# ami-iit/paper_gorbani_2025_humanoids_multi-rate-mpc-ironcub

Measured on AMD Instinct MI355X. Metric: MPC solves/sec (whole node) + p50 single-solve latency, iRonCub paper horizon, higher is better.
Workload: dtype f64

## Files before the change

paper_gorbani_2025_humanoids_multi-rate-mpc-ironcub_amd/csrc/vsmpc_p1_struct.hpp:

```cpp
#pragma once
#include "vsmpc_smem.hpp"

namespace vsmpc {

VS_DEV double uniform_f64(double x) {
    const int lo = __builtin_amdgcn_readfirstlane(__double2loint(x));
    const int hi = __builtin_amdgcn_readfirstlane(__double2hiint(x));
    return __hiloint2double(hi, lo);
}

template <class D, int KIND, bool SMALL = false>
VS_DEV void p1s_chain(const DevCfg& cfg, int half, int lane, double* __restrict__ sm) {
    using S = Smem<D, SMALL>;
    constexpr int N = D::N, HC = D::HC, NV = D::NV;
    const double* sA = sm + S::oA;
    const double* sCfg = sm + S::oCfg;
    double* sH = sm + S::oSH;
    double* sRb = sm + S::oSRb;
    double* sW3 = sm + S::oSW3;
    const int xr0 = half ? 6 : 0, hr0 = half ? 9 : 3, er0 = half ? 23 : 20;
    const int yx0 = half ? 6 : 0, yh0 = half ? 9 : 3, ye0 = half ? 15 : 12;
    double M1[9], qx[3], qh[3], qe[3];
#pragma unroll
    for (int r = 0; r < 3; ++r) {
// ... 120 lines not shown
                for (int r = 0; r < 3; ++r) {
                    rf_n[r] = refRow[rc * 12 + yx0 + r + zo];
                    rf_n[3 + r] = refRow[rc * 12 + yh0 + r + zo];
                }
            }
        }
        if (m < N) {
            const double dtm = cfg.dt[m];
            double t[3];
#pragma unroll
            for (int r = 0; r < 3; ++r) t[r] = fma(M1[6 + r], nx[2], fma(M1[3 + r], nx[1], M1[r] * nx[0]));
            t[0] = fma(-s02, nh[2], fma(-s01, nh[1], t[0]));
            t[1] = fma(-s12, nh[2], fma(s01, nh[0], t[1]));
            t[2] = fma(s12, nh[1], fma(s02, nh[0], t[2]));
#pragma unroll
            for (int r = 0; r < 3; ++r) {
                nx[r] = fma(dtm, ne[r], nx[r]);
                nh[r] = fma(dtm, t[r], nh[r]);
            }
        }
#pragma unroll
        for (int r = 0; r < 3; ++r) {
            nx[r] = fma(qx[r], KIND == 1 ? x[r] - rf[r] : x[r], nx[r]);
            nh[r] = fma(qh[r], KIND == 1 ? hk[i][r] - rf[3 + r] : hk[i][r], nh[r]);
            ne[r] = fma(qe[r], e[r], ne[r]);
        }
        const double dti = cfg.dt[i];
        if (m >= 2) {
            double hp[3] = {hk[i - 1][0], hk[i - 1][1], hk[i - 1][2]};
            asm volatile("" : "+v"(hp[0]), "+v"(hp[1]), "+v"(hp[2]));
#pragma unroll
            for (int r = 0; r < 3; ++r) {
                const double dxr = fma(M1[3 * r + 2], hp[2], fma(M1[3 * r + 1], hp[1], M1[3 * r] * hp[0]));
                x[r] = fma(-dti, dxr, x[r]);
                e[r] = fma(-dti, x[r], e[r]);
            }
        }
        double w[3];
#pragma unroll
        for (int a = 0; a < 3; ++a) { w[a] = dti * nh[a]; bs[a] += w[a]; }
        if constexpr (KIND == 1 && !LONG) {
            if (i >= 1 && live) {
                double* Wp = sW3 + ((half * (NV + 1) + col) * (N - 1) + (i - 1)) * 3;
#pragma unroll
                for (int a = 0; a < 3; ++a) Wp[a] = w[a];
            }
        }
        if constexpr (KIND == 1 && LONG) {
            if (i >= 1) {
                if (live && !isgen && i - 1 >= acFirst) {
                    typedef __attribute__((address_space(3))) double lds_double;
                    double* Ap = sm + S::oSAc + acOff + (i - 1) * 4;
#pragma unroll
                    for (int q = 0; q < NTH; ++q) {
                        const double v = fma(Am[2][q], w[2], fma(Am[1][q], w[1], Am[0][q] * w[0]));
                        __builtin_amdgcn_ds_atomic_fadd_f64((lds_double*)(Ap + q), v, 0, 0, false);
                    }
                }
            }
        }
        if (i < HC) {
            if (isgen) {
                if (live && i >= gb) {
                    double* Hp = sH + (half * D::NJPAIR + i * (i + 1) / 2 + gb) * 9 + gd;
#pragma unroll
                    for (int a = 0; a < 3; ++a) Hp[3 * a] = bs[a];
                }
            } else {
                if (live) {
                    double* Rp = sRb + ((half * (NV + 1) + col) * HC + i) * 3;
#pragma unroll
                    for (int a = 0; a < 3; ++a) Rp[a] = bs[a];
                }
            }
#pragma unroll
            for (int a = 0; a < 3; ++a) bs[a] = 0.0;
        }
        asm volatile("" : "+v"(nx[0]), "+v"(nx[1]), "+v"(nx[2]), "+v"(nh[0]), "+v"(nh[1]), "+v"(nh[2]), "+v"(ne[0]), "+v"(ne[1]), "+v"(ne[2]));
        asm volatile("" : "+v"(x[0]), "+v"(x[1]), "+v"(x[2]), "+v"(e[0]), "+v"(e[1]), "+v"(e[2]), "+v"(bs[0]), "+v"(bs[1]), "+v"(bs[2]));
        __builtin_amdgcn_sched_barrier(0);
    }
}

template <class D, bool SMALL = false>
VS_DEV void p1s_contract(double* __restrict__ sm, int tid) {
    using S = Smem<D, SMALL>;
    constexpr int NI = (D::NV + 1) * (D::N - 1);
    constexpr int ROUNDS = (NI + D::BLOCK - 1) / D::BLOCK;
    const double* sA = sm + S::oA;
    const double* sW3 = sm + S::oSW3;
    double* sAc = sm + S::oSAc;
    double w[ROUNDS][6];
#pragma unroll
    for (int rd = 0; rd < ROUNDS; ++rd) {
        const int ci = tid + rd * D::BLOCK, cic = ci < NI ? ci : NI - 1;
#pragma unroll
        for (int a = 0; a < 3; ++a) { w[rd][a] = sW3[cic * 3 + a]; w[rd][3 + a] = sW3[(NI + cic) * 3 + a]; }
    }
    double Am[6][NTH];
#pragma unroll
    for (int a = 0; a < 3; ++a)
#pragma unroll
        for (int q = 0; q < NTH; ++q) { Am[a][q] = sA[(3 + a) * NX + 12 + q]; Am[3 + a][q] = sA[(9 + a) * NX + 12 + q]; }
#pragma unroll
    for (int rd = 0; rd < ROUNDS; ++rd) {
        const int ci = tid + rd * D::BLOCK;
        double v[NTH];
#pragma unroll
        for (int q = 0; q < NTH; ++q) {
            v[q] = Am[0][q] * w[rd][0];
#pragma unroll
            for (int a = 1; a < 6; ++a) v[q] = fma(Am[a][q], w[rd][a], v[q]);
        }
        if (ci < NI) {
#pragma unroll
            for (int q = 0; q < NTH; ++q) sAc[ci * 4 + q] = v[q];
        }
    }
}

template <class D, int TPW, int W, bool PIPE>
struct AllSlots {
    static constexpr bool SMALL = false;
    static constexpr int count = TPW;
    static constexpr int slot(int a) { return a; }
    static constexpr bool forms(int q) { return TileTab<D, PIPE>{}.forms(q * D::NWAVES + W, W); }
};
template <class D, int TPW, int W, bool PIPE = false, class PLAN = AllSlots<D, TPW, W, PIPE>>
VS_DEV void p1s_entries(d4 (&acc)[TPW], const double* __restrict__ sm, int lane) {
    using S = Smem<D, PLAN::SMALL>;
    constexpr int PVT = D::PVT, N = D::N, HC = D::HC, NV = D::NV;
    static_assert(D::NU % 16 == 0, "joint rows are tile aligned");
    const double* sBj = sm + S::oBj;
    const double* sH = sm + S::oSH;
    const double* sRb = sm + S::oSRb;
    const double* sAc = sm + S::oSAc;
    const double* sJetT = sm + S::oJetT;
    lane = fresh_lane();
    const int j = lane & 15, g = lane >> 4;
    double Lq[3][NJC], LqM[3][NJC];
    int bin[3];
#pragma unroll
    for (int pat = 0; pat < 3; ++pat) {
        const int o = ((16 * pat) % NJC) + j;
        bin[pat] = o / NJC;
        const int un = o - NJC * bin[pat];
#pragma unroll
        for (int a6 = 0; a6 < NJC; ++a6) {
            Lq[pat][a6] = sBj[((a6 < 3 ? 3 : 6) + a6) * NJ + un];
            LqM[pat][a6] = bin[pat] == g ? Lq[pat][a6] : 0.0;
        }
    }
    constexpr int G = 3;
    constexpr int NSLOT = PLAN::count;
    constexpr int NGRP = (NSLOT + G - 1) / G;
    static_for<0, NGRP>([&](auto gcst) __attribute__((always_inline)) {
    constexpr int q0 = decltype(gcst)::value * G;
    constexpr int q1 = q0 + G < NSLOT ? q0 + G : NSLOT;
    double raw[G][NJC][3];
    static_for<q0, q1>([&](auto qcst) __attribute__((always_inline)) {
        constexpr TileTab<D, PIPE> tab{};
        constexpr int qi = decltype(qcst)::value;
        constexpr int q = PLAN::slot(qi);
        constexpr int t = q * D::NWAVES + W;
        if constexpr (PLAN::forms(q)) {
            constexpr int ti = tab.ti[t], tj = tab.tj[t];
            if constexpr (ti < PVT) {
                constexpr int b0r = (16 * ti) / NJC, b0c = (16 * tj) / NJC;
                const int brr = b0r + g, bcc = b0c + bin[tj % 3];
                const int br = brr < HC ? brr : HC - 1, bc = bcc < HC ? bcc : HC - 1;
                const bool sw = ti == tj && br < bc;
                const int hi = sw ? bc : br, lo = sw ? br : bc;
                const int st = sw ? 3 : 1, sa = sw ? 1 : 3;
                const double* Hp = sH + (hi * (hi + 1) / 2 + lo) * 9;
#pragma unroll
                for (int ks = 0; ks < NJC; ++ks) {
                    const double* Hk = Hp + (ks / 3) * D::NJPAIR * 9 + sa * (ks % 3);
#pragma unroll
                    for (int d = 0; d < 3; ++d) raw[qi - q0][ks][d] = Hk[d * st];
                }
            } else if constexpr (tj < PVT) {
                constexpr int b0c = (16 * tj) / NJC;
                const int cr = 16 * (ti - PVT) + j;
                const int crc = cr <= NV ? cr : NV;
                const int bcc = b0c + g, bc = bcc < HC ? bcc : HC - 1;
#pragma unroll
                for (int ks = 0; ks < NJC; ++ks)
                    raw[qi - q0][ks][0] = sRb[(((ks / 3) * (NV + 1) + crc) * HC + bc) * 3 + (ks % 3)];
            }
        }
    });
    __builtin_amdgcn_sched_barrier(0);
    double opa[G][NJC], opb[G][NJC];
    static_for<q0, q1>([&](auto qcst) __attribute__((always_inline)) {
        constexpr TileTab<D, PIPE> tab{};
        constexpr int qi = decltype(qcst)::value;
        constexpr int q = PLAN::slot(qi);
        constexpr int t = q * D::NWAVES + W;
#pragma unroll
        for (int ks = 0; ks < NJC; ++ks) { opa[qi - q0][ks] = 0.0; opb[qi - q0][ks] = 0.0; }
// ... 99 lines not shown
```

paper_gorbani_2025_humanoids_multi-rate-mpc-ironcub_amd/csrc/vsmpc_p3.hpp:

```cpp
#pragma once
#include "vsmpc_p1_struct.hpp"
#include "vsmpc_smem.hpp"

namespace vsmpc {

template <class D>
VS_DEV double input_cost_term(const double* __restrict__ sCfg, const double* __restrict__ sGy,
                              const double* __restrict__ sVprev, int gr, int gc) {
    if (gr < D::NU) return (gr == gc) ? 1.0 : 0.0;
    if (gr < D::NZ) {
        if (gc < D::NU) return 0.0;
        const int q1 = gr - D::NU, q2 = gc - D::NU;
        if ((q1 & 3) != (q2 & 3)) return 0.0;
        const int b1 = v_block_of_internal<D>(q1), b2 = v_block_of_internal<D>(q2);
        if (b1 == b2)
            return sCfg[CFG_WTHR] * double((b1 > 0) + (b1 < D::NVB - 1)) + (b1 == 0 ? sCfg[CFG_WINIT] : 0.0);
        const int db = b1 - b2;
        return (db == 1 || db == -1) ? -sCfg[CFG_WTHR] : 0.0;
    }
    if (gr == D::NZ && gc < D::NZ) {
        if (gc < D::NU) return gc < D::NUY ? sGy[gc % NJC] : 0.0;
        const int q = gc - D::NU;
        return v_block_of_internal<D>(q) == 0 ? -sCfg[CFG_WINIT] * sVprev[q & 3] : 0.0;
    }
// ... 264 lines not shown
                for (int ks = 0; ks < 4; ++ks)
                    acc[q0] = __builtin_amdgcn_mfma_f64_16x16x4f64(la[b][0][ks], lb[b][0][ks], acc[q0], 0, 0, 0);
            } else {
                d4 c2 = d4{0.0, 0.0, 0.0, 0.0};
                acc[q0] = __builtin_amdgcn_mfma_f64_16x16x4f64(la[b][0][0], lb[b][0][0], acc[q0], 0, 0, 0);
                c2 = __builtin_amdgcn_mfma_f64_16x16x4f64(la[b][0][1], lb[b][0][1], c2, 0, 0, 0);
                acc[q0] = __builtin_amdgcn_mfma_f64_16x16x4f64(la[b][0][2], lb[b][0][2], acc[q0], 0, 0, 0);
                c2 = __builtin_amdgcn_mfma_f64_16x16x4f64(la[b][0][3], lb[b][0][3], c2, 0, 0, 0);
#pragma unroll
                for (int r = 0; r < 4; ++r) acc[q0][r] += c2[r];
            }
            if constexpr (KIND != 2) {
                static_for<0, 2>([&](auto ucst) __attribute__((always_inline)) {
                    constexpr int u = decltype(ucst)::value;
                    if constexpr (a + u < n) {
                        constexpr int q = u ? q1 : q0;
                        double* T = sM + tile_off_c<D>(tab.ti[q * D::NWAVES + W], PP + 1) + crow;
#pragma unroll
                        for (int r = 0; r < 4; ++r) T[4 * r * 17] = acc[q][r];
                    }
                });
            }
        }
    });
}

VS_DEV void tile_inverse_dpp(const double* __restrict__ Lpp, const double* __restrict__ invd, double* __restrict__ X, int lane) {
    panel_inverse_dpp(lds_addr(Lpp + (lane & 15) * 17), lds_addr(invd), lds_addr(X + (lane & 15)), lane & 15);
}

template <class D, int TPW>
constexpr int pipe_inverse_wave(int p) {
    constexpr WaveLists<D, TPW, 1, true> w1{};
    constexpr WaveLists<D, TPW, 2, true> w2{};
    constexpr WaveLists<D, TPW, 3, true> w3{};
    const int n1 = w1.nrest[p - 1], n2 = w2.nrest[p - 1], n3 = w3.nrest[p - 1];
    return (n3 <= n1 && n3 <= n2) ? 3 : (n2 <= n1 ? 2 : 1);
}

template <class D, int TPW, int W, bool PIPE, class PLAN>
VS_DEV void p2_terms(const double* __restrict__ sCfg, d4 (&acc)[TPW], const double* __restrict__ sGy,
                     const double* __restrict__ sVprev, int lane) {
    constexpr TileTab<D, PIPE> tab{};
    constexpr int PVT = D::PVT;
    static_for<0, PLAN::count>([&](auto qcst) __attribute__((always_inline)) {
        constexpr int q = PLAN::slot(decltype(qcst)::value);
        constexpr int t = q * D::NWAVES + W;
        if constexpr (PLAN::forms(q)) {
            constexpr int ti = tab.ti[t], tj = tab.tj[t];
            if constexpr (ti == tj && 16 * ti + 16 <= D::NU) {
#pragma unroll
                for (int r = 0; r < 4; ++r) acc[q][r] += ((lane >> 4) + 4 * r == (lane & 15)) ? 1.0 : 0.0;
            } else if constexpr (ti >= PVT && 16 * tj + 16 <= D::NU) {
                if constexpr (ti == D::NT - 1) {
                    const int gc = 16 * tj + (lane & 15);
                    const double gv = sGy[gc % NJC];
                    const double gq = gc < D::NUY ? gv : 0.0;
#pragma unroll
                    for (int r = 0; r < 4; ++r) acc[q][r] += (16 * ti + (lane >> 4) + 4 * r == D::NZ) ? gq : 0.0;
                }
            } else if constexpr (ti == tj || ti >= PVT) {
#pragma unroll
                for (int r = 0; r < 4; ++r)
                    acc[q][r] += input_cost_term<D>(sCfg, sGy, sVprev, 16 * ti + (lane >> 4) + 4 * r, 16 * tj + (lane & 15));
            }
        }
    });
}

constexpr int SMALL_BESIDE0 = 4;
template <class D>
constexpr bool small_wave0_forms(int ti) {
    return ti % (D::NWAVES - 1) == 0 && ti / (D::NWAVES - 1) < (D::NT + 1) / 4;
}
template <class D, int TPW, int W>
constexpr int small_instalment(int q) {
    constexpr TileTab<D, true> tab{};
    const int t = q * D::NWAVES + W;
    if (!tab.ok(t)) return -1;
    if (W == 0) return small_wave0_forms<D>(tab.ti[t]) ? 0 : -1;
    if (tab.tj[t] == 0) return (W == 1 && small_wave0_forms<D>(tab.ti[t])) ? -1 : 0;
    int n = 0;
    for (int b = 0; b < q; ++b) n += (tab.ok(b * D::NWAVES + W) && tab.tj[b * D::NWAVES + W] > 0) ? 1 : 0;
    return (tab.tj[t] == 1 || n < SMALL_BESIDE0) ? 1 : 2;
}
template <class D, int TPW, int W, int INST>
struct SmallPlan {
    static constexpr bool SMALL = true;
    static constexpr int count_() {
        int n = 0;
        for (int q = 0; q < TPW; ++q) n += small_instalment<D, TPW, W>(q) == INST ? 1 : 0;
        return n;
    }
    static constexpr int count = count_();
    static constexpr int slot(int a) {
        for (int q = 0; q < TPW; ++q)
            if (small_instalment<D, TPW, W>(q) == INST && a-- == 0) return q;
        return 0;
    }
    static constexpr bool forms(int) { return true; }
};
template <class D, int TPW>
constexpr bool small_plan_complete() {
    constexpr TileTab<D, true> tab{};
    int col0[D::NT] = {};
    for (int q = 0; q < TPW; ++q) {
        const int i0 = small_instalment<D, TPW, 0>(q);
        if (i0 >= 0) col0[tab.ti[q * D::NWAVES]] += 1;
        const int inst[3] = {small_instalment<D, TPW, 1>(q), small_instalment<D, TPW, 2>(q), small_instalment<D, TPW, 3>(q)};
        for (int w = 1; w < D::NWAVES; ++w) {
            const int t = q * D::NWAVES + w;
            if (!tab.ok(t)) continue;
            if (tab.tj[t] == 0) col0[tab.ti[t]] += inst[w - 1] == 0 ? 1 : 0;
            else if (inst[w - 1] < 1) return false;
        }
    }
    for (int i = 0; i < D::NT; ++i)
        if (col0[i] != 1) return false;
    return true;
}
template <class D, int TPW, int W, int INST>
VS_DEV void small_form(const double* __restrict__ sCfg, d4 (&acc)[TPW], double* __restrict__ sM, const double* __restrict__ sGy,
                       const double* __restrict__ sVprev, int lane, int crow) {
    using PLAN = SmallPlan<D, TPW, W, INST>;
    static_assert(small_plan_complete<D, TPW>(), "every tile is formed exactly once");
    if constexpr (PLAN::count > 0) {
        p1s_entries<D, TPW, W, true, PLAN>(acc, sM - Smem<D>::oM, lane);
        p2_terms<D, TPW, W, true, PLAN>(sCfg, acc, sGy, sVprev, lane);
        if constexpr (INST == 0) {
            constexpr TileTab<D, true> tab{};
            static_for<0, PLAN::count>([&](auto acst) __attribute__((always_inline)) {
                constexpr int q = PLAN::slot(decltype(acst)::value);
                double* T = sM + tile_off_c<D>(tab.ti[q * D::NWAVES + W], 0) + crow;
#pragma unroll
                for (int r = 0; r < 4; ++r) T[4 * r * 17] = acc[q][r];
            });
        }
    }
}

template <class D, int TPW, int W, bool DEBUG, bool PIPE = false, bool SMALL = false>
VS_DEV void cholesky_wave(const double* __restrict__ sCfg, d4 (&acc)[TPW], double* __restrict__ sM, double* __restrict__ sInvD,
                          const double* __restrict__ sGy, const double* __restrict__ sVprev, int* __restrict__ sFlags,
                          double* __restrict__ sXinv, double* __restrict__ sW, double* __restrict__ dbgL, int lane,
                          int crow, int lrow, double* sZ_) {
    constexpr TileTab<D, PIPE> tab{};
    constexpr WaveLists<D, TPW, W, PIPE> wl{};
    using S = Smem<D>;
    constexpr int PVT = D::PVT;
    constexpr int GL = D::NZ & 15;
    if constexpr (D::WG_PER_CU == 1) pin_tiles_agpr<TPW>(acc);
    if constexpr (!SMALL) p2_terms<D, TPW, W, PIPE, AllSlots<D, TPW, W, PIPE>>(sCfg, acc, sGy, sVprev, lane);
    if constexpr (D::WG_PER_CU == 1) pin_tiles_agpr<TPW>(acc);
#pragma unroll
    for (int q = 0; q < TPW; ++q) {
        const int t = q * D::NWAVES + W;
        if (!SMALL && tab.forms(t, W) && tab.tj[t] == 0) {
            double* T = sM + tile_off_c<D>(tab.ti[t], 0) + crow;
#pragma unroll
            for (int r = 0; r < 4; ++r) T[4 * r * 17] = acc[q][r];
        }
    }
    __syncthreads();
#ifdef VS_DIAG_P3
    unsigned long long p3_mark = __builtin_amdgcn_s_memtime();
    if (DEBUG && W == 0 && lane < 4) vs_diag_p3[lane] = 0;
#endif
    if constexpr (PIPE) {
        constexpr bool ND = D::WG_PER_CU == 1;
        static_for<0, D::NT>([&](auto pcst) __attribute__((always_inline)) {
            constexpr int p = decltype(pcst)::value;
            if constexpr (D::WG_PER_CU == 1) pin_tiles_agpr<TPW>(acc);
            constexpr int below = D::NP - 16 * p - 16;
            constexpr int nshare0 = (below + 63) / 64;
            constexpr int SL = below <= 64 ? 1 : (below <= 128 ? 2 : 3);
            static_assert(p == 0 ? nshare0 <= D::NWAVES - 1 : below <= 192, "rows of a panel fit the streams");
            double* scratch = p <= PVT ? sXinv + p * D::TS + 64 * W : sZ_ + 64 * W;
            double diag[16];
            if constexpr (p == D::NT - 1) {
                constexpr int NPIV_LAST = D::NZ - 16 * (D::NT - 1);
                if constexpr (NPIV_LAST == 8 || NPIV_LAST == 12) {
                    if (W == 0 && panel_last_dpp<D, NPIV_LAST>(sM, sInvD, lane) && lane == 0) sFlags[0] = 1;
                } else {
                    if (W == 0 && panel_factor<D, NPIV_LAST>(sM, sInvD, p, lane) && lane == 0) sFlags[0] = 1;
                }
            } else if constexpr (p == 0 && SMALL) {
                static_assert(!SMALL || nshare0 <= 3, "row slots of one stream");
                if constexpr (W == 0) {
                    if (panel_dpp<D, nshare0>(sM, sInvD, p, lane, 0, diag, scratch) && lane == 0) sFlags[0] = 1;
                } else {
                    small_form<D, TPW, W, 1>(sCfg, acc, sM, sGy, sVprev, lane, crow);
                }
            } else if constexpr (p == 0) {
                if (W < nshare0) {
                    const int bad = panel_dpp<D, 1>(sM, sInvD, p, lane, W, diag, scratch);
                    if (W == 0 && bad && lane == 0) sFlags[0] = 1;
                }
            } else if constexpr (W == 0) {
                constexpr int KB = !ND ? 0 : (SL == 3 ? 6 : (SL == 1 ? 3 : (pipe_max_others<D, TPW, p - 1>() > 2 ? 6 : 3)));
                int bad;
                if constexpr (16 * p + 16 == D::NU && D::NU - D::NUY == 8 && SL == 1 && KB == 0)
                    bad = panel_dummy_dpp<D, p>(sM, sInvD, lane, diag, scratch);
                else
                    bad = panel_dpp<D, SL, KB>(sM, sInvD, p, lane, 0, diag, scratch);
                if (bad && lane == 0) sFlags[0] = 1;
            }
            auto park_next_diag = [&]() __attribute__((always_inline)) {
                if constexpr (ND && W >= 1 && p + 1 < D::NT - 1) {
                    static_for<0, TPW>([&](auto qcst) __attribute__((always_inline)) {
                        constexpr int q = decltype(qcst)::value;
                        constexpr int t = q * D::NWAVES + W;
                        if constexpr (tab.holds(t, W)) {
                            if constexpr (tab.ti[t] == p + 1 && tab.tj[t] == p + 1) {
                                double* T = sM + (S::oNextDiag - S::oM) + crow;
#pragma unroll
                                for (int r = 0; r < 4; ++r) T[4 * r * 17] = acc[q][r];
                            }
                        }
                    });
                }
            };
            if constexpr (p == 0) park_next_diag();
            if constexpr (p >= 1 && W >= 1) {
                if constexpr (SMALL && p == 1) small_form<D, TPW, W, 2>(sCfg, acc, sM, sGy, sVprev, lane, crow);
                if constexpr (p - 1 < PVT) {
#pragma unroll
                    for (int q = 0; q < TPW; ++q) {
                        const int t = q * D::NWAVES + W;
                        if (tab.holds(t, W) && tab.tj[t] == p - 1 && tab.ti[t] > p - 1) {
                            const double* T = sM + tile_off_c<D>(tab.ti[t], p - 1) + crow;
#pragma unroll
                            for (int r = 0; r < 4; ++r) acc[q][r] = T[4 * r * 17];
                            if (tab.ti[t] == D::NT - 1 && (lane >> 4) == (GL & 3)) sW[16 * (p - 1) + (lane & 15)] = -acc[q][GL >> 2];
                        }
                    }
                }
                pipe_update<D, TPW, W, p - 1, 2>(acc, sM, lrow, crow);
                park_next_diag();
                if constexpr (W == pipe_inverse_wave<D, TPW>(p)) {
                    if constexpr (p - 1 < S::NXT)
                        tile_inverse_dpp(sM + tile_off_c<D>(p - 1, p - 1), sInvD + 16 * (p - 1), sXinv + (p - 1) * D::TS, lane);
                    if constexpr (S::DUAL3 && p - 1 == D::PVT + 1)
                        tile_inverse_dpp(sM + tile_off_c<D>(p - 1, p - 1), sInvD + 16 * (p - 1), sM + (S::oDual3T0 - S::oM), lane);
                }
            }
            VS_P3_MARK(0);
// ... 136 lines not shown
```

paper_gorbani_2025_humanoids_multi-rate-mpc-ironcub_amd/csrc/vsmpc_smem.hpp:

```cpp
#pragma once
#include <type_traits>

#include "vsmpc_device.hpp"

namespace vsmpc {

typedef double d4 __attribute__((ext_vector_type(4)));

template <class D, bool PIPE = false>
__device__ constexpr TileTab<D, PIPE> kTileTab{};
template <class D>
__device__ constexpr NactTab<D> kNactTab{};
template <class D>
__device__ constexpr TilePack<D> kTilePack{};

template <int I, int N, class F>
VS_DEV void static_for(F&& f) {
    if constexpr (I < N) {
        f(std::integral_constant<int, I>{});
        static_for<I + 1, N>(f);
    }
}

VS_DEV int fresh_lane() {
    unsigned m = ~0u;
    asm volatile("" : "+s"(m));
    return int(__builtin_amdgcn_mbcnt_hi(m, __builtin_amdgcn_mbcnt_lo(m, 0u)));
}

template <class D, bool SMALL = false>
struct Smem {
    static constexpr bool DUALQP = D::NT - 2 == D::PVT && D::NU % 16 == 0 && D::NV >= 20 && D::NV <= 32;
    static constexpr int oIn = 0;
    static constexpr int oA = oIn + ((D::NIN + 3) & ~3);
    static constexpr int oBj = oA + NX * NX;
    static constexpr int oBt = oBj + NX * NJ;
    static constexpr int oC = oBt + NX * NTH;
    static constexpr int oVprev = oC + 28;
    static constexpr int oInvD = oVprev + 4;
    static constexpr int oW = oInvD + D::NP;
    static constexpr int oZ = oW + D::NP;
    static constexpr int oSvec = oZ + D::NP;
    static constexpr int oV = oSvec + D::NV;
    static constexpr int oDt = oV + D::NV;
    static constexpr int oCfg = oDt + MAX_STAGES;
    static constexpr int oFlags = oCfg + CFG_SIZE;
    static constexpr int NFLAGS = 5;
    static_assert(NFLAGS * sizeof(int) <= 4 * sizeof(double), "the int flags fit their four doubles (oQR follows)");
    static constexpr int oQR = (oFlags + 4 + 3) & ~3;
    static constexpr int QR_V = 0, QR_BETA = 48, QR_GY = 56, QR_NS = 62, QR_ISW = 64, QR_A = 72, QR_SIZE = 128;
    static constexpr int NXT = D::PVT + 1;
    static constexpr int oXinv = (oQR + QR_SIZE + 3) & ~3;
    static constexpr int oR = oXinv + NXT * D::TS;
    static constexpr int YROWS = 36;
    static constexpr int oY = oR;
    static constexpr int sizeY = YROWS * D::YS;
    static constexpr int oM = oR;
    static constexpr int sizeM = D::L_TILES * D::TS;
    static constexpr int NVS = D::NV + 1;
    static constexpr int oSv = oR;
    static constexpr bool DUAL3 = !DUALQP && D::NT - 3 == D::PVT && D::NU % 16 == 0 && D::NV > 32 && D::NV <= 48;
    static constexpr int oQP = oSv + D::NV * NVS;
    static constexpr int sizeQP = DUALQP ? D::NV * NVS + (D::NV - 16) * NVS : (DUAL3 ? 2 * D::NV * NVS + 2 * D::TS : 0);
    static constexpr int oDual3T0 = oQP + 2 * D::NV * NVS;
    static constexpr int oDual3T1 = oDual3T0 + D::TS;
    static constexpr int oU = DUAL3 ? oR : oQP + sizeQP;
    static constexpr int oX = oU + D::NWAVES * D::NP;
    static constexpr int oF = oX + D::NXS;
    static constexpr int endScratch = (oF + NX * D::N > oQP + sizeQP) ? oF + NX * D::N : oQP + sizeQP;
    static_assert(endScratch <= oR + D::CORNER_TILE0 * D::TS, "P4..P6 scratch must not reach the corner tiles");
    static constexpr int NJROW = D::NV + NTH + 1;
    static constexpr int oP1Small = ((oR + D::L_TILES * D::TS + D::TS > endScratch ? oR + D::L_TILES * D::TS + D::TS : endScratch) + 3) & ~3;
    static constexpr int oJetT = SMALL ? oP1Small : oXinv;
    static constexpr int oGA = oJetT + NJROW * D::N;
    static constexpr int oSH = oGA + 6 * D::N;
    static constexpr int oSRb = oSH + 2 * D::NJPAIR * 9;
    static constexpr int oSW3 = oSRb + 2 * (D::NV + 1) * D::HC * 3;
    static constexpr int oSAc = oSW3 + (D::STRUCT_LONG ? 0 : 2 * (D::NV + 1) * (D::N - 1) * 3);
    static constexpr int AC_SHORT = D::STRUCT_LONG ? D::NV - NTH : 0;
    static constexpr int AC_NSH = D::STRUCT_LONG ? D::NS : 0;
    VS_HD static constexpr int ac_first(int cr) { return cr < AC_SHORT ? AC_NSH : 0; }
    VS_HD static constexpr int ac_off(int cr) {
        return 4 * (cr * (D::N - 1) - (cr < AC_SHORT ? cr : AC_SHORT) * AC_NSH);
    }
    static constexpr int sizeAc = ac_off(D::NV + 1);
    static constexpr int oSRefC = oSAc + sizeAc;
    static constexpr int sizeZero = 3 * D::N > 12 * D::NREF ? 3 * D::N : 12 * D::NREF;
    static constexpr int oSZero = D::STRUCT_LONG ? oW : oSRefC + 12 * D::NREF;
    static_assert(!D::STRUCT_LONG || sizeZero <= 2 * D::NP, "zeros fit the w and z vectors");
    static constexpr int endP1s = D::STRUCT_LONG ? oSRefC + 12 * D::NREF : oSZero + sizeZero;
    static constexpr int oNextDiag = oM + sizeM;
    static constexpr int total_syrk = oR + (sizeY > sizeM ? sizeY : sizeM);
    static constexpr int total_struct = D::STRUCT_P1 ? (endP1s > oNextDiag + D::TS ? endP1s : oNextDiag + D::TS) : total_syrk;
    static constexpr int total = total_syrk;
    static constexpr size_t bytes = size_t(total) * sizeof(double);
    static constexpr size_t bytes_struct = size_t(total_struct) * sizeof(double);
    static_assert(bytes <= 160 * 1024 && bytes_struct <= 160 * 1024, "LDS budget of one CU");
    static_assert(SMALL || D::WG_PER_CU < 2 || (bytes <= 80 * 1024 && bytes_struct <= 80 * 1024), "two workgroups per CU");
    static_assert(!SMALL || (D::STRUCT_P1 && !D::STRUCT_LONG), "the small-batch kind exists for short structured horizons");
    static_assert(!SMALL || (oJetT >= oNextDiag + D::TS && oJetT >= endScratch && oJetT >= oXinv + NXT * D::TS && endP1s <= total_struct),
                  "small-batch kind: the arrays of P1 stay apart from everything P3..P6 write");
};

template <class D>
constexpr bool has_small_kind() { return D::STRUCT_P1 && !D::STRUCT_LONG && D::WG_PER_CU == 2; }

template <class D>
VS_HD constexpr int tile_off_c(int i, int j) {
    return (j < D::PVT ? (j & 1) * D::RING_A + (i - j)
                       : D::CORNER_TILE0 + (i - D::PVT) * (i - D::PVT + 1) / 2 + (j - D::PVT)) * D::TS;
}
template <class D>
VS_DEV int tile_off(int i, int j) { return tile_off_c<D>(i, j); }

template <class D>
VS_DEV int lower_at(int gr, int gc) {
    return tile_off<D>(gr >> 4, gc >> 4) + (gr & 15) * 17 + (gc & 15);
}

}
```

paper_gorbani_2025_humanoids_multi-rate-mpc-ironcub_amd/csrc/vsmpc_solve_body.inc:

```
#define VS_STAMP(i)                                                                        \
    do {                                                                                    \
        if constexpr (STAMPS) {                                                             \
            unsigned long long* st_ = late_args()->stamps;                                  \
            if (tid == 0 && st_ != nullptr) st_[size_t(blockIdx.x) * 16 + (i)] = __builtin_amdgcn_s_memtime(); \
        }                                                                                   \
    } while (0)
    unsigned long long t_acc[6] = {0, 0, 0, 0, 0, 0};
    unsigned long long t_mark = 0, stamp_t1 = 0, rt0 = 0;
    if constexpr (STAMPS) rt0 = __builtin_amdgcn_s_memrealtime();
#define VS_TIC()                                                     \
    do {                                                             \
        if constexpr (STAMPS) t_mark = __builtin_amdgcn_s_memtime(); \
    } while (0)
#define VS_TOC(i)                                                          \
    do {                                                                   \
        if constexpr (STAMPS) {                                            \
            const unsigned long long t_now = __builtin_amdgcn_s_memtime(); \
            t_acc[i] += t_now - t_mark;                                    \
            t_mark = t_now;                                                \
        }                                                                  \
    } while (0)
    using S = Smem<D, SMALL>;
    static_assert(!SMALL || (FORM == 1 && !TUNED), "the small-batch kind is the structured form of the shared kind");
    constexpr bool PIPE = FORM == 1;
// ... 84 lines not shown
    constexpr int NJROW = D::NV + NTH + 1, ZROW = D::NV + NTH;
    double* sJetT = sXinv;
    if constexpr (SMALL) sJetT = smem + S::oJetT;
    static_assert(SMALL || S::oJetT == S::oXinv, "the jet trajectories lie at the head of the X region");
    double* sGA = sJetT + NJROW * D::N;
    static_assert(D::NV + NTH <= 64 && (SMALL || NJROW * D::N + 6 * D::N <= S::NXT * D::TS), "jet trajectories fit the X region");
    if (wave == 1) {
        if (lane < D::NV + NTH) {
            const bool affl = lane >= D::NV;
            const int i = affl ? lane - D::NV : (lane & 3);
            const int blk = affl ? -1 : v_block_of_internal<D>(lane);
            const double jon = sA[(12 + i) * NX + 16 + i], ja = sA[(16 + i) * NX + 12 + i], jb = sA[(16 + i) * NX + 16 + i];
            const double c12 = sC[12 + i], c16 = sC[16 + i], b12 = sBt[(12 + i) * NTH + i], b16 = sBt[(16 + i) * NTH + i];
            const double t0 = sIn[VSMPC_IN_X0 + 12 + i], td0 = sIn[VSMPC_IN_X0 + 16 + i];
            const double bT = affl ? c12 : b12, bTd = affl ? c16 : b16;
            double T = affl ? t0 : 0.0, Td = affl ? td0 : 0.0;
#pragma unroll
            for (int k = 0; k < D::N; ++k) {
                sJetT[lane * D::N + k] = T;
                const double mT = (affl || throttle_block_of_stage<D>(k) == blk) ? 1.0 : 0.0;
                const double dT = fma(jon, Td, mT * bT);
                const double dTd = fma(ja, T, fma(jb, Td, mT * bTd));
                const double dt = sDt[k];
                T = fma(dt, dT, T);
                Td = fma(dt, dTd, Td);
            }
        }
        for (int k = lane; k < D::N; k += 64) sJetT[ZROW * D::N + k] = 0.0;
        if constexpr (FORM == 1) {
            const double am = sIn[VSMPC_IN_ALPHA] * sIn[VSMPC_IN_MASS];
            const double* R = sIn + VSMPC_IN_WRB;
            const double* gr = sIn + VSMPC_IN_GRAV;
            for (int e = lane; e < 6 * D::N; e += 64) {
                const int h = e / (3 * D::N), k = (e / 3) % D::N, r = e % 3;
                double g = 0.0;
#pragma unroll
                for (int c = 0; c < NTH; ++c) g = fma(sIn[VSMPC_IN_AMOM + (3 * h + r) * NTH + c], sJetT[(D::NV + c) * D::N + k], g);
                const double ch = h == 0 ? am * (R[0 + r] * gr[0] + R[3 + r] * gr[1] + R[6 + r] * gr[2]) : 0.0;
                sGA[e] = g + ch;
            }
        }
    }
    if constexpr (FORM == 1) {
        if (wave == 2) {
            for (int e = lane; e < S::sizeZero; e += 64) smem[S::oSZero + e] = 0.0;
            for (int e = lane; e < 12 * D::NREF; e += 64) {
                const int row = e % 12;
                const double off = row < 3 ? -sIn[VSMPC_IN_PREF + row] : ((row >= 6 && row < 9) ? -sIn[VSMPC_IN_RPYINIT + row - 6] : 0.0);
                smem[S::oSRefC + e] = sIn[VSMPC_IN_XREF + e] + off;
            }
        }
    }
    if constexpr (FORM == 1 && D::STRUCT_LONG) {
        for (int e = tid; e < S::sizeAc; e += D::BLOCK) smem[S::oSAc + e] = 0.0;
    }
    __syncthreads();
    if constexpr (FORM != 1) {
        for (int e = tid; e < 6 * D::N; e += D::BLOCK) {
            const int h = e / (3 * D::N), k = (e / 3) % D::N, r = e % 3, row = (h ? 9 : 3) + r;
            double g = 0.0;
#pragma unroll
            for (int c = 0; c < NTH; ++c) g = fma(sA[row * NX + 12 + c], sJetT[(D::NV + c) * D::N + k], g);
            sGA[e] = g;
        }
        __syncthreads();
    }

    VS_STAMP(1);
    VS_REFRESH_IDS();
    if constexpr (STAMPS) stamp_t1 = __builtin_amdgcn_s_memtime();
    d4 acc[TPW];
    if constexpr (FORM == 1) {
        static_assert(D::STRUCT_P1, "structured condensing is instantiated for horizons with Dims::STRUCT_P1");
        VS_TIC();
        if (wave < 2) {
            p1s_chain<D, 0, SMALL>(cfg, wave, lane, smem);
            if (wave == 0) p0_joint_reduction<D, QR_P0_STEPS, NJC>(smem, lane);
        } else {
            p1s_chain<D, 1, SMALL>(cfg, wave - 2, lane, smem);
        }
        VS_TOC(0);
        __syncthreads();
        VS_TOC(1);
        if constexpr (!D::STRUCT_LONG) {
            p1s_contract<D, SMALL>(smem, tid);
            __syncthreads();
        }
        VS_TOC(3);
        auto tail = [&](auto wcst) __attribute__((always_inline)) {
            constexpr int W = decltype(wcst)::value;
            if constexpr (SMALL) {
                static_for<0, TPW>([&](auto qcst) __attribute__((always_inline)) {
                    constexpr int q = decltype(qcst)::value;
                    if constexpr (small_instalment<D, TPW, W>(q) < 0) acc[q] = d4{0.0, 0.0, 0.0, 0.0};
                });
                const int ln0 = fresh_lane();
                small_form<D, TPW, W, 0>(sCfg, acc, Lb, smem + S::oQR + S::QR_GY, sVprev, ln0, (ln0 >> 4) * 17 + (ln0 & 15));
            } else {
                p1s_entries<D, TPW, W, PIPE>(acc, smem, lane);
            }
            VS_TOC(2);
            __syncthreads();
            VS_STAMP(2);
            constexpr TileTab<D, PIPE> tab{};
            double* dbgLw = nullptr;
            if constexpr (STAMPS && !SMALL) {
                double* dbgM = late_args()->dbgM;
                double* dbgL = late_args()->dbgL;
                dbgLw = dbgL != nullptr ? dbgL + size_t(inst) * D::NP * D::NP : nullptr;
                if (dbgM != nullptr) {
                    const int ln = fresh_lane();
                    static_for<0, TPW>([&](auto qcst) __attribute__((always_inline)) {
                        constexpr int q = decltype(qcst)::value;
                        constexpr int t = q * D::NWAVES + W;
                        if constexpr (tab.forms(t, W))
                            dump_hessian_tile<D>(dbgM + size_t(inst) * D::NP * D::NP, tab.ti[t], tab.tj[t], acc[q], sCfg,
                                                 smem + S::oQR + S::QR_GY, sVprev, ln);
                    });
                }
            }
            VS_STAMP(3);
            if constexpr (D::WG_PER_CU == 1) pin_tiles_agpr<TPW>(acc);
            const int ln = fresh_lane();
            cholesky_wave<D, TPW, W, STAMPS, PIPE, SMALL>(sCfg, acc, Lb, sInvD, smem + S::oQR + S::QR_GY, sVprev, sFlags, sXinv, sW, dbgLw, ln,
                                                  (ln >> 4) * 17 + (ln & 15), (ln & 15) * 17 + (ln >> 4), sZ);
            if constexpr (STAMPS) {
                if (dbgLw != nullptr) {
                    const int l2 = fresh_lane();
                    static_for<0, TPW>([&](auto qcst) __attribute__((always_inline)) {
                        constexpr int q = decltype(qcst)::value;
                        constexpr int t = q * D::NWAVES + W;
                        if constexpr (tab.holds(t, W) && tab.tj[t] < D::PVT && tab.ti[t] > tab.tj[t])
                            dump_factor_tile<D>(dbgLw, tab.ti[t], tab.tj[t], acc[q], l2);
                    });
                }
            }
        };
        switch (wave) {
            case 0: tail(std::integral_constant<int, 0>{}); break;
            case 1: tail(std::integral_constant<int, 1>{}); break;
            case 2: tail(std::integral_constant<int, 2>{}); break;
            default: tail(std::integral_constant<int, 3>{}); break;
        }
    } else {
#pragma unroll
        for (int q = 0; q < TPW; ++q) acc[q] = d4{0.0, 0.0, 0.0, 0.0};
        constexpr int CPT = D::CPT;
        const int pw = wave;
        const int ptid = tid;
        const int half = pw / (D::NWAVES / 2);
        const int xr0 = half ? 6 : 0, hr0 = half ? 9 : 3, er0 = half ? 23 : 20;
        const int yx0 = half ? 6 : 0, yh0 = half ? 9 : 3, ye0 = half ? 15 : 12;

        double M1[9], Sk[9], Ce[3], sqx[3], sqh[3], sqe[3];
        auto load_coeffs = [&]() __attribute__((always_inline)) {
#pragma unroll
            for (int r = 0; r < 3; ++r) {
#pragma unroll
                for (int c = 0; c < 3; ++c) {
                    M1[3 * r + c] = sA[(xr0 + r) * NX + hr0 + c];
                    Sk[3 * r + c] = sA[(hr0 + r) * NX + hr0 + c];
                }
                Ce[r] = sC[er0 + r];
                sqx[r] = sCfg[CFG_SQ + yx0 + r];
                sqh[r] = sCfg[CFG_SQ + yh0 + r];
                sqe[r] = sCfg[CFG_SQ + ye0 + r];
            }
        };
// ... 682 lines not shown
```

Baseline: 8.484 million.

## Overlap sAc contraction with tile forming in small-batch kind, dropping a barrier

In the small-batch kernel, the sAc contraction no longer runs as a separate phase followed by a block barrier. Waves 1-3 now compute it at the start of their instalment-1 tile forming, while wave 0 runs its own stream. Tiles that read sAc (both indices at or above PVT) are forced into instalment 2, which comes after a later barrier, and a compile-time check enforces this. The aim is to remove one __syncthreads and hide the contraction behind other work, at the cost of fewer threads doing the contraction and more instalment-2 tiles. One other barrier is also skipped for SMALL, and the small kind is restricted to PVT>=2.

```diff
diff --git a/paper_gorbani_2025_humanoids_multi-rate-mpc-ironcub_amd/csrc/vsmpc_p1_struct.hpp b/paper_gorbani_2025_humanoids_multi-rate-mpc-ironcub_amd/csrc/vsmpc_p1_struct.hpp
--- a/paper_gorbani_2025_humanoids_multi-rate-mpc-ironcub_amd/csrc/vsmpc_p1_struct.hpp
+++ b/paper_gorbani_2025_humanoids_multi-rate-mpc-ironcub_amd/csrc/vsmpc_p1_struct.hpp
@@ -226,9 +226,9 @@
     }
 }
 
-template <class D, bool SMALL = false>
+template <class D>
 VS_DEV void p1s_contract(double* __restrict__ sm, int tid) {
-    using S = Smem<D, SMALL>;
+    using S = Smem<D>;
     constexpr int NI = (D::NV + 1) * (D::N - 1);
     constexpr int ROUNDS = (NI + D::BLOCK - 1) / D::BLOCK;
     const double* sA = sm + S::oA;
@@ -260,6 +260,41 @@
 #pragma unroll
             for (int q = 0; q < NTH; ++q) sAc[ci * 4 + q] = v[q];
         }
+    }
+}
+
+template <class D>
+VS_DEV void p1s_contract_beside(double* __restrict__ sm, int t) {
+    using S = Smem<D, true>;
+    constexpr int NI = (D::NV + 1) * (D::N - 1);
+    constexpr int NTHR = (D::NWAVES - 1) * 64;
+    constexpr int ROUNDS = (NI + NTHR - 1) / NTHR;
+    const double* sA = sm + S::oA;
+    const double* sW3 = sm + S::oSW3;
+    double* sAc = sm + S::oSAc;
+    double Am[6][NTH];
+#pragma unroll
+    for (int a = 0; a < 3; ++a)
+#pragma unroll
+        for (int q = 0; q < NTH; ++q) { Am[a][q] = sA[(3 + a) * NX + 12 + q]; Am[3 + a][q] = sA[(9 + a) * NX + 12 + q]; }
+#pragma unroll
+    for (int rd = 0; rd < ROUNDS; ++rd) {
+        const int ci = t + rd * NTHR, cic = ci < NI ? ci : NI - 1;
+        double w[6];
+#pragma unroll
+        for (int a = 0; a < 3; ++a) { w[a] = sW3[cic * 3 + a]; w[3 + a] = sW3[(NI + cic) * 3 + a]; }
+        double v[NTH];
+#pragma unroll
+        for (int q = 0; q < NTH; ++q) {
+            v[q] = Am[0][q] * w[0];
+#pragma unroll
+            for (int a = 1; a < 6; ++a) v[q] = fma(Am[a][q], w[a], v[q]);
+        }
+        if (ci < NI) {
+#pragma unroll
+            for (int q = 0; q < NTH; ++q) sAc[ci * 4 + q] = v[q];
+        }
+        __builtin_amdgcn_sched_barrier(0);
     }
 }
 
diff --git a/paper_gorbani_2025_humanoids_multi-rate-mpc-ironcub_amd/csrc/vsmpc_p3.hpp b/paper_gorbani_2025_humanoids_multi-rate-mpc-ironcub_amd/csrc/vsmpc_p3.hpp
--- a/paper_gorbani_2025_humanoids_multi-rate-mpc-ironcub_amd/csrc/vsmpc_p3.hpp
+++ b/paper_gorbani_2025_humanoids_multi-rate-mpc-ironcub_amd/csrc/vsmpc_p3.hpp
@@ -370,6 +370,7 @@
     if (tab.tj[t] == 0) return (W == 1 && small_wave0_forms<D>(tab.ti[t])) ? -1 : 0;
     int n = 0;
     for (int b = 0; b < q; ++b) n += (tab.ok(b * D::NWAVES + W) && tab.tj[b * D::NWAVES + W] > 0) ? 1 : 0;
+    if (tab.ti[t] >= D::PVT && tab.tj[t] >= D::PVT) return 2;
     return (tab.tj[t] == 1 || n < SMALL_BESIDE0) ? 1 : 2;
 }
 template <class D, int TPW, int W, int INST>
@@ -407,11 +408,29 @@
         if (col0[i] != 1) return false;
     return true;
 }
+template <class D, int TPW>
+constexpr bool small_ac_tiles_last() {
+    constexpr TileTab<D, true> tab{};
+    for (int q = 0; q < TPW; ++q) {
+        const int inst[D::NWAVES] = {small_instalment<D, TPW, 0>(q), small_instalment<D, TPW, 1>(q), small_instalment<D, TPW, 2>(q),
+                                     small_instalment<D, TPW, 3>(q)};
+        for (int w = 0; w < D::NWAVES; ++w) {
+            const int t = q * D::NWAVES + w;
+            if (inst[w] >= 0 && tab.ti[t] >= D::PVT && tab.tj[t] >= D::PVT && inst[w] != 2) return false;
+        }
+    }
+    return true;
+}
 template <class D, int TPW, int W, int INST>
 VS_DEV void small_form(const double* __restrict__ sCfg, d4 (&acc)[TPW], double* __restrict__ sM, const double* __restrict__ sGy,
                        const double* __restrict__ sVprev, int lane, int crow) {
     using PLAN = SmallPlan<D, TPW, W, INST>;
     static_assert(small_plan_complete<D, TPW>(), "every tile is formed exactly once");
+    static_assert(small_ac_tiles_last<D, TPW>(), "the tiles that read sAc are formed behind the barrier that publishes it");
+    if constexpr (INST == 1) {
+        static_assert(W >= 1, "wavefront 0 runs stream 0 meanwhile");
+        p1s_contract_beside<D>(sM - Smem<D>::oM, 64 * (W - 1) + lane);
+    }
     if constexpr (PLAN::count > 0) {
         p1s_entries<D, TPW, W, true, PLAN>(acc, sM - Smem<D>::oM, lane);
         p2_terms<D, TPW, W, true, PLAN>(sCfg, acc, sGy, sVprev, lane);
@@ -449,7 +468,7 @@
             for (int r = 0; r < 4; ++r) T[4 * r * 17] = acc[q][r];
         }
     }
-    __syncthreads();
+    if constexpr (!SMALL) __syncthreads();
 #ifdef VS_DIAG_P3
     unsigned long long p3_mark = __builtin_amdgcn_s_memtime();
     if (DEBUG && W == 0 && lane < 4) vs_diag_p3[lane] = 0;
diff --git a/paper_gorbani_2025_humanoids_multi-rate-mpc-ironcub_amd/csrc/vsmpc_smem.hpp b/paper_gorbani_2025_humanoids_multi-rate-mpc-ironcub_amd/csrc/vsmpc_smem.hpp
--- a/paper_gorbani_2025_humanoids_multi-rate-mpc-ironcub_amd/csrc/vsmpc_smem.hpp
+++ b/paper_gorbani_2025_humanoids_multi-rate-mpc-ironcub_amd/csrc/vsmpc_smem.hpp
@@ -103,7 +103,7 @@
 };
 
 template <class D>
-constexpr bool has_small_kind() { return D::STRUCT_P1 && !D::STRUCT_LONG && D::WG_PER_CU == 2; }
+constexpr bool has_small_kind() { return D::STRUCT_P1 && !D::STRUCT_LONG && D::WG_PER_CU == 2 && D::PVT >= 2; }
 
 template <class D>
 VS_HD constexpr int tile_off_c(int i, int j) {
diff --git a/paper_gorbani_2025_humanoids_multi-rate-mpc-ironcub_amd/csrc/vsmpc_solve_body.inc b/paper_gorbani_2025_humanoids_multi-rate-mpc-ironcub_amd/csrc/vsmpc_solve_body.inc
--- a/paper_gorbani_2025_humanoids_multi-rate-mpc-ironcub_amd/csrc/vsmpc_solve_body.inc
+++ b/paper_gorbani_2025_humanoids_multi-rate-mpc-ironcub_amd/csrc/vsmpc_solve_body.inc
@@ -190,8 +190,8 @@
         VS_TOC(0);
         __syncthreads();
         VS_TOC(1);
-        if constexpr (!D::STRUCT_LONG) {
-            p1s_contract<D, SMALL>(smem, tid);
+        if constexpr (!D::STRUCT_LONG && !SMALL) {
+            p1s_contract<D>(smem, tid);
             __syncthreads();
         }
         VS_TOC(3);
```

New measurement: 8.586 million, median of 6. 1.01x the previous value.
